# may-/joeys2t

Measured on AMD Instinct MI355X. Metric: audio frames/sec (train step, 80-mel, 15 s utt, bs32 per GPU), higher is better.
Workload: dtype bf16; 1 GPU; configs/librispeech_100h.yaml ASR train step on synthetic 16 kHz waveforms; global_batch=32, frames_per_utt=1498, encoder_len=375, lengths=fixed 15 s, vocab=5000, batch_multiplier=1, parallelism=dp1, launch=hipGraph replay

## Files before the change

include/joeys2t_hip.h:

```cpp
#ifndef JOEYS2T_HIP_H
#define JOEYS2T_HIP_H

#include <stdint.h>

#ifdef __cplusplus
extern "C" {
#endif

typedef void* js2t_stream;

enum { JS2T_F32 = 0, JS2T_BF16 = 1, JS2T_FP8_E4M3 = 2  };
enum { JS2T_ACT_NONE = 0, JS2T_ACT_RELU = 1, JS2T_ACT_GELU = 2, JS2T_ACT_SWISH = 3, JS2T_ACT_TANH = 4, JS2T_ACT_HARDSWISH = 5 };
enum { JS2T_OK = 0, JS2T_ERR_INVALID = -1, JS2T_ERR_LAUNCH = -2, JS2T_ERR_UNSUPPORTED = -3 };

int js2t_abi_version(void);
const char* js2t_last_error(void);

typedef struct js2t_gemm_desc {
  int32_t M, N, K;
  int32_t batch, batch_inner;
  int32_t dtype_ab, dtype_c;
  int32_t trans_a, trans_b;
  const void* A; int64_t lda, a_stride_o, a_stride_i;
  const void* B; int64_t ldb, b_stride_o, b_stride_i;
// ... 43 lines not shown
void js2t_gemm_p192_mode(int mode);
void js2t_gemm_wg256_mode(int mode);
void js2t_gemm_p192_ring(int nst);
void js2t_gemm_panel_mode(int mode);


int js2t_axpby(const void* x, float a, const void* y, float b, void* out, int64_t n, int dt, js2t_stream stream);

int js2t_cast(const void* src, int src_dt, void* dst, int dst_dt, int64_t n, js2t_stream stream);

int js2t_fold_ln_weights(const int64_t* table, int32_t n_entries, int32_t max_rows, js2t_stream stream);

int js2t_absmax(const void* x, int dt, int64_t n, float* out, js2t_stream stream);
int js2t_quantize_fp8(const void* x, int dt, void* y, int64_t n, const float* amax, const float* mul, float* scale_out,
                      js2t_stream stream);
int js2t_quantize_fp8_delayed(const void* x, int dt, void* y, int64_t n, float* state, const float* mul, float* scale_out,
                              js2t_stream stream);

int js2t_glu_fwd(const void* x, void* y, int64_t rows, int64_t C, int dt, js2t_stream stream);
int js2t_glu_bwd(const void* x, const void* dy, void* dx, int64_t rows, int64_t C, int dt, js2t_stream stream);
int js2t_glu_fwd_crop(const void* x, void* y, int64_t rows, int64_t C, int64_t T, const int64_t* valid_t, int dt, js2t_stream stream);
int js2t_glu_bwd_crop(const void* x, const void* dy, void* dx, int64_t rows, int64_t C, int64_t T, const int64_t* valid_t, int dt,
                      js2t_stream stream);

int js2t_transpose_groups(const void* src, void* dst, const int64_t* table, int32_t n_groups, int64_t total_tiles, js2t_stream stream);

int js2t_add_pe_dropout(const void* x, const float* pe, const void* extra, void* y, int64_t B, int64_t T,
                        int64_t D, int dt, float p, const uint64_t* rng_state, uint32_t rng_stream,
                        js2t_stream stream);

int js2t_dropout_bwd(const void* dy, void* dx, int64_t rows, int64_t cols, int dt, float p,
                     const uint64_t* rng_state, uint32_t rng_stream, js2t_stream stream);

int js2t_act_bwd(const void* dh, const void* z, void* dz, int64_t n, int act, int dt, float scale,
                 js2t_stream stream);

int js2t_embed_fwd(const int64_t* ids, const void* table, int table_dt, void* out, int out_dt,
                   int64_t n_ids, int64_t D, int64_t vocab, float scale, js2t_stream stream);
int js2t_embed_bwd(const int64_t* ids, const void* dout, int dout_dt, float* dtable, int64_t n_ids,
                   int64_t D, int64_t vocab, float scale, int64_t pad_idx, js2t_stream stream);

int64_t js2t_colsum_partial_rows(int64_t rows);
int js2t_colsum(const void* x, int dt, float* out, float* partial, int64_t rows, int64_t cols, int accumulate,
                js2t_stream stream);

int js2t_pack_rows(const void* src, void* dst, const int32_t* seg, int32_t B, int32_t T, int64_t rows_out, int64_t row_bytes,
// ... 212 lines not shown
```

joeys2t_amd/builders.py:

```python
from typing import Callable

from torch import nn


class ConfigurationError(Exception):
    """Custom exception for misspecifications of configuration (reference config.py:22)."""


class _Tanh(nn.Module):
    def forward(self, x):
        raise RuntimeError("placeholder activation module: the HIP GEMM epilogue applies tanh")


_ACTIVATIONS = {"relu": nn.ReLU, "gelu": nn.GELU, "tanh": _Tanh, "swish": nn.SiLU}


def build_activation(activation: str = "relu") -> Callable:
    try:
        return _ACTIVATIONS[activation]
    except KeyError:
        raise ConfigurationError("Invalid activation function. Valid options: " + ", ".join(repr(k) for k in _ACTIVATIONS) + ".") from None


import ctypes as _C
# ... 129 lines not shown
                    _C.c_float(g["weight_decay"]), _C.c_int64(self.t), ops._p(coef), _C.c_float(grad_scale), int(zero_grad),
                    ops._p(lr_dev), ops._p(step_dev), ops._stream())
            for table, n_items, n_units in plan["launches"]:
                check(lib().js2t_adamw_items(ops._p(st.flat), ops._p(st.flat_grad), ops._p(self.exp_avg), ops._p(self.exp_avg_sq),
                                             ops._p(lp), ops._p(st.flat_lp_t if lp is not None else None), ops._p(table),
                                             _C.c_int32(n_items), _C.c_int64(n_units), ops._p(plan["folds"]), *args), "js2t_adamw_items")
            ops.WEIGHT_VERSION += 1
            st.dirty = lp is None and st.dirty
            if plan["left_folds"] is not None:
                ops.fold_ln_weights(plan["left_folds"], plan["left_folds"].shape[0], plan["left_max_rows"])
            return
        for lo, hi in self.update_ranges:
            check(lib().js2t_adamw(_off(st.flat, lo), _off(st.flat_grad, lo), _off(self.exp_avg, lo), _off(self.exp_avg_sq, lo),
                                   _off(lp, lo), _C.c_int64(hi - lo), _C.c_float(g["lr"]), _C.c_float(g["betas"][0]),
                                   _C.c_float(g["betas"][1]), _C.c_float(g["eps"]), _C.c_float(g["weight_decay"]), _C.c_int64(self.t),
                                   ops._p(coef), _C.c_float(grad_scale), int(zero_grad), ops._p(lr_dev), ops._p(step_dev),
                                   ops._stream()), "js2t_adamw")
        ops.WEIGHT_VERSION += 1
        st.dirty = lp is None and st.dirty
        if lp is not None and st.flat_lp_t is not None:
            st.refresh_t()
        if lp is not None:
            st.refresh_folds()

    def _fused_plan(self):
        st = self.store
        if not FUSED_UPDATE or self.update_ranges != [(0, st.total)]:
            return None
        key = (len(st._fold_rows), st.flat_lp is not None, st.flat_lp_t is not None, None if self.keep is None else self.keep.version)
        if self._plan_key == key:
            return self._plan
        if torch.cuda.is_current_stream_capturing():
            raise RuntimeError("FlatAdamW: the store changed (new LayerNorm folds / shadows) after the last eager update: "
                               "run one eager step before capturing")
        if self._plan is not None:
            self._retired_plans.append(self._plan)
            self.plan_generation += 1
        self._plan_key, self._plan = key, None
        from joeys2t_amd._lib import lib
        geo = [_C.c_int32() for _ in range(3)]
        lib().js2t_adamw_items_geometry(*[_C.byref(v) for v in geo])
        flat_unit, unit_rows, unit_cols = (int(v.value) for v in geo)
        mats = sorted((off, R, Cc) for off, R, Cc, _ in st._tgroups)
        if any(Cc % 4 or off % 4 for off, R, Cc in mats):
            return None
        base = st.flat.data_ptr()
        fold_of, left = {}, []
        for i, row in enumerate(st._fold_rows):
            hit = [(off, R, Cc) for off, R, Cc in mats if base + 4 * off == row[0] and R == row[6] and Cc == row[7]]
            if hit and row[7] <= unit_cols and hit[0][0] not in fold_of:
                fold_of[hit[0][0]] = i
            else:
                left.append(row)
        small, big, pos = [], [], 0
        for off, R, Cc in mats:
            if off > pos:
                small.append([0, pos, off - pos, 1, 0, -1, 0, 0])
            kept = int(self.keep is not None and self.keep.contains(off, off + R * Cc))
            big.append([1, off, R, Cc, 0, fold_of.get(off, -1), kept, 0])
            pos = off + R * Cc
        if st.total > pos:
            small.append([0, pos, st.total - pos, 1, 0, -1, 0, 0])
        launches = []
        for items in (small, big):
            if not items:
                continue
            units = 0
            for it in items:
                it[4] = units
                units += -(-it[2] // flat_unit) if it[0] == 0 else -(-it[2] // unit_rows) * -(-it[3] // unit_cols)
            launches.append((torch.tensor(items, dtype=torch.int64, device=st.device), len(items), units))
        folds = torch.tensor(st._fold_rows, dtype=torch.int64, device=st.device) if st._fold_rows else None
        self._plan = {"launches": launches, "folds": folds,
                      "left_folds": torch.tensor(left, dtype=torch.int64, device=st.device) if left else None,
                      "left_max_rows": max((r[6] for r in left), default=0)}
        return self._plan

    def state_dict(self) -> Dict:
        return {"t": self.t, "exp_avg": self.exp_avg, "exp_avg_sq": self.exp_avg_sq, "param_groups": self.param_groups}

    def load_state_dict(self, sd: Dict):
        self.t = sd["t"]
        self.exp_avg.copy_(sd["exp_avg"])
        self.exp_avg_sq.copy_(sd["exp_avg_sq"])
        self.param_groups = sd["param_groups"]
        self.step_dev.fill_(self.t)
        self.lr_dev.fill_(self.param_groups[0]["lr"])

    def torch_state_dict(self, params) -> Dict:
        st = self.store
        state = {}
        if self.t > 0:
            for i, p in enumerate(params):
# ... 59 lines not shown
```

joeys2t_amd/csrc/elementwise.hip:

```cpp
#include "common.hpp"

namespace {

constexpr int EW_THREADS = 256;
inline int ew_grid(int64_t work_items) {
  int64_t g = (work_items + EW_THREADS - 1) / EW_THREADS;
  if (g < 1) g = 1;
  if (g > 4096) g = 4096;
  return (int)g;
}

template <typename T> struct vec4;
template <> struct vec4<float> {
  static __device__ __forceinline__ void ld(const float* p, float (&v)[4]) {
    const float4 x = *(const float4*)p; v[0] = x.x; v[1] = x.y; v[2] = x.z; v[3] = x.w;
  }
  static __device__ __forceinline__ void st(float* p, const float (&v)[4]) {
    *(float4*)p = make_float4(v[0], v[1], v[2], v[3]);
  }
};
template <> struct vec4<uint16_t> {
  static __device__ __forceinline__ void ld(const uint16_t* p, float (&v)[4]) {
    const uint2 x = *(const uint2*)p;
    v[0] = __uint_as_float(x.x << 16); v[1] = __uint_as_float(x.x & 0xffff0000u);
    v[2] = __uint_as_float(x.y << 16); v[3] = __uint_as_float(x.y & 0xffff0000u);
  }
  static __device__ __forceinline__ void st(uint16_t* p, const float (&v)[4]) {
    uint2 x;
    x.x = pack_bf16x2(v[0], v[1]);
    x.y = pack_bf16x2(v[2], v[3]);
    *(uint2*)p = x;
  }
};

template <typename S, typename D>
__global__ void cast_kernel(const S* __restrict__ src, D* __restrict__ dst, int64_t n) {
  const int64_t n4 = n >> 2;
  for (int64_t i = blockIdx.x * (int64_t)blockDim.x + threadIdx.x; i < n4; i += (int64_t)gridDim.x * blockDim.x) {
    float v[4];
    vec4<S>::ld(src + 4 * i, v);
    vec4<D>::st(dst + 4 * i, v);
  }
  for (int64_t i = (n4 << 2) + blockIdx.x * (int64_t)blockDim.x + threadIdx.x; i < n; i += (int64_t)gridDim.x * blockDim.x)
    io<D>::st(dst + i, io<S>::ld(src + i));
}

template <typename T>
__global__ void axpby_kernel(const T* __restrict__ x, float a, const T* __restrict__ y, float b, T* __restrict__ out,
                             int64_t n) {
  for (int64_t i = blockIdx.x * (int64_t)blockDim.x + threadIdx.x; i < n; i += (int64_t)gridDim.x * blockDim.x) {
    float v = a * io<T>::ld(x + i);
    if (y) v += b * io<T>::ld(y + i);
    io<T>::st(out + i, v);
  }
}

// ... 142 lines not shown
  const int cl = threadIdx.x & 63, sub = threadIdx.x >> 6;
  const int64_t c = ((int64_t)blockIdx.x * 64 + cl) * 8;
  const int64_t r0 = (int64_t)blockIdx.y * CS_ROWS_PER_BLOCK, r1 = min(rows, r0 + CS_ROWS_PER_BLOCK);
  float s[8] = {0.f, 0.f, 0.f, 0.f, 0.f, 0.f, 0.f, 0.f};
  if (c < cols)
    for (int64_t r = r0 + sub; r < r1; r += 4) {
      const uint4 v = *(const uint4*)(x + r * cols + c);
      const uint32_t vv[4] = {v.x, v.y, v.z, v.w};
#pragma unroll
      for (int i = 0; i < 4; ++i) {
        s[2 * i] += __uint_as_float(vv[i] << 16);
        s[2 * i + 1] += __uint_as_float(vv[i] & 0xffff0000u);
      }
    }
#pragma unroll
  for (int i = 0; i < 8; ++i) sh[sub][cl][i] = s[i];
  __syncthreads();
  if (sub == 0 && c < cols) {
#pragma unroll
    for (int i = 0; i < 8; ++i)
      partial[(int64_t)blockIdx.y * cols + c + i] = (sh[0][cl][i] + sh[1][cl][i]) + (sh[2][cl][i] + sh[3][cl][i]);
  }
}
__global__ __launch_bounds__(256) void colsum_final_kernel(const float* __restrict__ partial, float* __restrict__ out, int64_t nparts,
                                                           int64_t cols, int accumulate) {
  __shared__ float sh[4][64];
  const int cl = threadIdx.x & 63, sub = threadIdx.x >> 6;
  const int64_t c = (int64_t)blockIdx.x * 64 + cl;
  float s0 = 0.f, s1 = 0.f;
  if (c < cols) {
    int64_t p = sub;
    for (; p + 4 < nparts; p += 8) {
      s0 += partial[p * cols + c];
      s1 += partial[(p + 4) * cols + c];
    }
    for (; p < nparts; p += 4) s0 += partial[p * cols + c];
  }
  sh[sub][cl] = s0 + s1;
  __syncthreads();
  if (sub == 0 && c < cols) {
    const float tot = (sh[0][cl] + sh[1][cl]) + (sh[2][cl] + sh[3][cl]);
    out[c] = accumulate ? out[c] + tot : tot;
  }
}

template <typename D>
// ... 259 lines not shown
                           js2t_stream stream) {
  if (cols == 0) return JS2T_OK;
  if (rows == 0) {
    JS2T_CHECK(out, "colsum: bad arguments");
    if (!accumulate) {
      hipError_t e = hipMemsetAsync(out, 0, sizeof(float) * cols, (hipStream_t)stream);
      JS2T_CHECK(e == hipSuccess, "colsum: memset failed: %s", hipGetErrorString(e));
    }
    return JS2T_OK;
  }
  JS2T_CHECK(x && out && partial && rows > 0, "colsum: bad arguments");
  const int64_t nparts = js2t_colsum_partial_rows(rows);
  JS2T_CHECK(nparts <= 65535, "colsum: too many rows");
  hipStream_t s = (hipStream_t)stream;
  if (dt == JS2T_BF16 && cols % 8 == 0 && (((uintptr_t)x) & 15) == 0) {
    hipLaunchKernelGGL(colsum_partial_vec_kernel, dim3(cdiv(cols, 512), (unsigned)nparts), dim3(256), 0, s, (const uint16_t*)x,
                       partial, rows, cols);
  } else {
    const dim3 g1(cdiv(cols, 64), (unsigned)nparts);
    DISPATCH_DT(dt, T, hipLaunchKernelGGL((colsum_partial_kernel<T>), g1, dim3(256), 0, s, (const T*)x, partial, rows, cols));
  }
  JS2T_LAUNCH_CHECK();
  hipLaunchKernelGGL(colsum_final_kernel, dim3(cdiv(cols, 64)), dim3(256), 0, s, partial, out, nparts, cols, accumulate);
  JS2T_LAUNCH_CHECK();
  return JS2T_OK;
}

extern "C" int js2t_conv_weight_pack(const float* w, void* wp, int wp_dt, int64_t cout, int64_t cin, int64_t k,
                                     js2t_stream stream) {
  JS2T_CHECK(w && wp && cout > 0 && cin > 0 && k > 0, "conv_weight_pack: bad arguments");
  DISPATCH_DT(wp_dt, D, hipLaunchKernelGGL((conv_pack_kernel<D>), dim3(ew_grid(cout * cin * k)), dim3(EW_THREADS), 0,
                                           (hipStream_t)stream, w, (D*)wp, cout, cin, k));
  JS2T_LAUNCH_CHECK();
  return JS2T_OK;
}
extern "C" int js2t_conv_weight_unpack_grad(const float* dwp_t, float* dw, int64_t cout, int64_t cin, int64_t k,
                                            int accumulate, js2t_stream stream) {
  JS2T_CHECK(dwp_t && dw && cout > 0 && cin > 0 && k > 0, "conv_weight_unpack_grad: bad arguments");
  hipLaunchKernelGGL(conv_unpack_grad_kernel, dim3(ew_grid(cout * cin * k)), dim3(EW_THREADS), 0, (hipStream_t)stream, dwp_t,
                     dw, cout, cin, k, accumulate);
  JS2T_LAUNCH_CHECK();
  return JS2T_OK;
}
extern "C" int js2t_col2im(const void* dcol, void* dx, int64_t B, int64_t tin, int64_t tout, int64_t C, int64_t K,
                           int64_t stride, int64_t pad, int dt, js2t_stream stream) {
  if (B * tin * C == 0) return JS2T_OK;
// ... 271 lines not shown
```

joeys2t_amd/csrc/optim.hip:

```cpp
#include "common.hpp"

namespace {

constexpr int SQ_BLOCK = 256;
constexpr int SQ_PER_BLOCK = 256 * 16 * 4;

__global__ __launch_bounds__(SQ_BLOCK) void sumsq_partial_kernel(const float* __restrict__ x, int64_t n, float* __restrict__ partial) {
  __shared__ float red[SQ_BLOCK / 64];
  const int64_t base = (int64_t)blockIdx.x * SQ_PER_BLOCK;
  const int64_t end = min(n, base + SQ_PER_BLOCK);
  float s = 0.f;
  for (int64_t i = base + threadIdx.x * 4; i < end; i += SQ_BLOCK * 4) {
    if (i + 4 <= end) {
      const float4 v = *(const float4*)(x + i);
      s += v.x * v.x + v.y * v.y + v.z * v.z + v.w * v.w;
    } else {
      for (int64_t j = i; j < end; ++j) s += x[j] * x[j];
    }
  }
  s = block_sum(s, red);
  if (threadIdx.x == 0) partial[blockIdx.x] = s;
}


// ... 93 lines not shown
                                                          float wd, float bc1, float bc2_sqrt, const float* __restrict__ gscale_dev,
                                                          float gscale, int zero_grad, const float* __restrict__ lr_dev,
                                                          const int64_t* __restrict__ step_dev) {
  extern __shared__ __attribute__((aligned(16))) uint16_t tile[];
  AdamConsts k;
  k.gs = gscale * (gscale_dev ? *gscale_dev : 1.f);
  if (lr_dev) lr = *lr_dev;
  if (step_dev) {
    const double t = (double)(*step_dev);
    bc1 = (float)(1.0 - pow((double)b1, t));
    bc2_sqrt = (float)sqrt(1.0 - pow((double)b2, t));
  }
  k.lr = lr, k.b1 = b1, k.b2 = b2, k.eps = eps, k.wd = wd, k.bc2_sqrt = bc2_sqrt, k.step_size = lr / bc1;
  const int64_t bid = blockIdx.x;
  int lo = 0, hi = n_items - 1;
  while (lo < hi) {
    const int mid = (lo + hi + 1) >> 1;
    if (items[mid * 8 + 4] <= bid) lo = mid; else hi = mid - 1;
  }
  const int64_t* it = items + 8 * lo;
  const int64_t kind = it[0], off = it[1], R = it[2], Cc = it[3], u = bid - it[4], fold = it[5];
  if (it[6]) zero_grad = 0;
  const float4 zero4 = make_float4(0.f, 0.f, 0.f, 0.f);
  if (kind == 0) {
    const int64_t base = off + u * ADAM_FLAT, end = min(off + R, base + (int64_t)ADAM_FLAT);
    for (int64_t i = base + threadIdx.x * 4; i < end; i += 1024) {
      const float4 pv = *(float4*)(p + i), gv = *(float4*)(g + i), mv = *(float4*)(m + i), vv = *(float4*)(v + i);
      float pa[4] = {pv.x, pv.y, pv.z, pv.w}, ma[4] = {mv.x, mv.y, mv.z, mv.w}, va[4] = {vv.x, vv.y, vv.z, vv.w};
      adam4(pa, gv, ma, va, k);
      *(float4*)(p + i) = make_float4(pa[0], pa[1], pa[2], pa[3]);
      *(float4*)(m + i) = make_float4(ma[0], ma[1], ma[2], ma[3]);
      *(float4*)(v + i) = make_float4(va[0], va[1], va[2], va[3]);
      if (zero_grad) *(float4*)(g + i) = zero4;
      if (lp) *(uint2*)(lp + i) = make_uint2(pack_bf16x2(pa[0], pa[1]), pack_bf16x2(pa[2], pa[3]));
    }
    return;
  }
  const int64_t chunks = (Cc + ADAM_COLS - 1) / ADAM_COLS;
  const int64_t strip = u / chunks, r0 = strip * ADAM_ROWS, c0 = (u - strip * chunks) * ADAM_COLS;
  const int wave = threadIdx.x >> 6, lane = threadIdx.x & 63;
  const int64_t* fe = (fold >= 0 && chunks == 1) ? folds + 8 * fold : nullptr;
  float4 gam[2] = {zero4, zero4}, bet[2] = {zero4, zero4};
  if (fe) {
#pragma unroll
    for (int j = 0; j < 2; ++j) {
      const int64_t c = 4 * lane + 256 * j;
      if (c < Cc) gam[j] = *(const float4*)((const float*)fe[1] + c), bet[j] = *(const float4*)((const float*)fe[2] + c);
    }
  }
#pragma unroll 2
  for (int rr = 0; rr < ADAM_ROWS / 4; ++rr) {
    const int lr_ = wave * (ADAM_ROWS / 4) + rr;
    const int64_t r = r0 + lr_;
    if (r >= R) break;
    float pn[2][4];
    float cs = 0.f, bs = 0.f;
#pragma unroll
// ... 137 lines not shown
```

joeys2t_amd/encoders.py:

```python
import os
from typing import List, Tuple

import torch
from torch import Tensor, nn

from joeys2t_amd import functional as Fn
from joeys2t_amd import ops
from joeys2t_amd.helpers import freeze_params, lengths_to_padding_mask, pad
from joeys2t_amd.runtime import runtime_of
from joeys2t_amd.transformer_layers import ConformerEncoderLayer, PositionalEncoding, TransformerEncoderLayer


PACK_RAGGED = os.environ.get("JS2T_PACKED_ENCODER", "1") != "0"
PACK_MIN_SAVING = 0.04
PACK_ROUND = 64
_PACK_CACHE: dict = {}


class Encoder(nn.Module):

    @property
    def output_size(self):
        return self._output_size

# ... 12 lines not shown
    def get_out_seq_lens_tensor(self, in_seq_lens_tensor: Tensor) -> Tensor:
        out = in_seq_lens_tensor.long()
        for k in self.kernel_sizes:
            out = torch.div(out + 2 * (k // 2) - k, 2, rounding_mode="floor") + 1
        return out

    def out_len(self, t_in: int) -> int:
        for k in self.kernel_sizes:
            t_in = Fn.conv_out_len(t_in, k)
        return t_in

    def forward(self, src_tokens: Tensor, src_lengths: Tensor, crop: Tensor = None) -> Tuple[Tensor, Tensor, Tensor]:
        rt = runtime_of(self)
        if not src_lengths.is_cuda:
            max_len = int(src_lengths.max())
            assert max_len > 0, "empty batch!"
            if src_tokens.size(1) != max_len:
                src_tokens = src_tokens[:, :max_len, :]
            src_lengths = src_lengths.to(src_tokens.device)
        x = rt.act_in(src_tokens.contiguous())
        for i, conv in enumerate(self.conv_layers):
            valid = crop[i:i + 1] if (crop is not None and i + 1 < self.n_layers) else None
            x = Fn.Conv1dGluFn.apply(x, conv.weight, conv.bias, rt.compute_dtype,
                                     rt.sinks({"w": [conv.weight], "b": [conv.bias]}), rt.grads_ready, valid)
        out_lens, mask = ops.subsample_lengths_mask(src_lengths, x.size(1), self.kernel_sizes)
        mask.js2t_row_sums = out_lens
        return x, out_lens, mask


class TransformerEncoder(Encoder):

    def __init__(self, hidden_size: int = 512, ff_size: int = 2048, num_layers: int = 8, num_heads: int = 4,
                 dropout: float = 0.1, emb_dropout: float = 0.1, freeze: bool = False, **kwargs):
        super().__init__()
        self._output_size = hidden_size
        self.layers = nn.ModuleList([
            TransformerEncoderLayer(size=hidden_size, ff_size=ff_size, num_heads=num_heads, dropout=dropout,
                                    alpha=kwargs.get("alpha", 1.0), layer_norm=kwargs.get("layer_norm", "pre"),
                                    activation=kwargs.get("activation", "relu")) for _ in range(num_layers)
        ])
        self.pe = PositionalEncoding(hidden_size)
        self.emb_dropout = nn.Dropout(p=emb_dropout)
        self.layer_norm = nn.LayerNorm(hidden_size, eps=1e-6) if kwargs.get("layer_norm", "post") == "pre" else None
        if freeze:
            freeze_params(self)
        self.subsample = kwargs.get("subsample", False)
        if self.subsample:
# ... 110 lines not shown
```

joeys2t_amd/functional.py:

```python
import math
from typing import List, Optional

import os

import torch

from joeys2t_amd import ops
from joeys2t_amd.ops import DropoutRng

LN_EPS = 1e-6


def _row_major_2d(t: torch.Tensor) -> torch.Tensor:
    if t.dim() != 2 or t.stride(1) != 1:
        raise ops.Js2tError(f"expected a row-major 2-D tensor, got shape {tuple(t.shape)} strides {t.stride()}")
    return t


FP8_FORWARD = os.environ.get("JS2T_FP8_FORWARD", "0") == "1"
FP8_SEPARATE_PASS = os.environ.get("JS2T_FP8_SEPARATE_PASS", "0") == "1"
_FP8_WEIGHTS = {}
_FP8_STATES = {}
FP8_DELAYED = os.environ.get("JS2T_FP8_DELAYED", "1") != "0"

# ... 840 lines not shown

        dz, dw2, db2 = linear_bwd(dy2, z, w2c, dw_out=sv("w2", w2c), db_out=sink.get("b2"), queue=sink.get("_wq"))
        dv, dgamma, dbeta = ops.bn_act_bwd(dz, v2, gamma, beta, mean, invstd, training, "hardswish")
        du, dwd = ops.dwconv_outer_bwd(dv.view(B, T, -1), u.view(B, T, -1), wd2)
        dbd = ops.colsum(dv)
        dh = ops.glu_bwd(h, du.view(B * T, -1))
        dx, dw1, db1 = linear_bwd(dh, x2, w1c, dw_out=sv("w1", w1c), db_out=sink.get("b1"), queue=sink.get("_wq"))
        if sink and ctx.notify is not None:
            ctx.notify(ctx.leaves)
        dx = dx.view(B, T, Cc)
        if dx.dtype != in_dtype:
            dx = dx.to(in_dtype)
        return (dx, None if dw1 is None else dw1.view(dw1.shape[0], Cc, 1), db1, dwd.view(dwd.shape[0], 1, -1), dbd, dgamma, dbeta, None, None,
                None if dw2 is None else dw2.view(dw2.shape[0], -1, 1), db2, None, None, None, None, None, None, None, None)


def conv_out_len(t_in: int, k: int, stride: int = 2) -> int:
    return (t_in + 2 * (k // 2) - (k - 1) - 1) // stride + 1


class Conv1dGluFn(torch.autograd.Function):

    @staticmethod
    def forward(ctx, x, weight, bias, compute_dtype, sink=None, notify=None, valid_t=None):
        ctx.sink, ctx.notify, ctx.leaves = sink, notify, (weight, bias)
        ctx.valid_t = valid_t
        B, T, Cin = x.shape
        Cout, _, K = weight.shape
        stride, pad = 2, K // 2
        Tout = conv_out_len(T, K, stride)
        x = x.contiguous()
        wp = ops.conv_weight_pack(weight, compute_dtype)
        M = B * Tout
        pre = torch.empty((M, Cout), dtype=compute_dtype, device=x.device)
        conv = (T, Tout, Cin, stride, pad)
        vec = 8 if x.dtype == torch.bfloat16 else 4
        if Cin % vec == 0:
            col = ops.im2col(x, K, stride, pad, Tout)
            ops.gemm(col, wp, pre, M=M, N=Cout, K=K * Cin, lda=K * Cin, ldb=K * Cin, ldc=Cout, bias=bias)
        else:
            col = None
            ops.gemm(x, wp, pre, M=M, N=Cout, K=K * Cin, lda=stride * Cin, ldb=K * Cin, ldc=Cout, bias=bias, conv=conv)
        y = ops.glu_fwd(pre, Tout, valid_t)
        ctx.x, ctx.wp, ctx.pre, ctx.conv, ctx.col = (x if col is None else None), wp, pre, conv, col
        ctx.dims = (B, T, Cin, Cout, K, Tout)
        return y.view(B, Tout, Cout // 2)

    @staticmethod
    def backward(ctx, dy):
        B, T, Cin, Cout, K, Tout = ctx.dims
        M = B * Tout
        x, wp, pre, conv = ctx.x, ctx.wp, ctx.pre, ctx.conv
        dy2 = dy.reshape(M, Cout // 2)
        if not dy2.is_contiguous():
            dy2 = dy2.contiguous()
        dpre = ops.glu_bwd(pre, dy2, Tout, ctx.valid_t)
        sink = ctx.sink or {}
        db = ops.colsum(dpre, out=sink.get("b"), accumulate=True) if sink else ops.colsum(dpre)
        sk = wgrad_split(K * Cin, Cout, M)
        dwp_t = (torch.zeros if sk > 1 else torch.empty)((K * Cin, Cout), dtype=torch.float32, device=dpre.device)
        if ctx.col is not None:
            ops.gemm(ctx.col, dpre, dwp_t, M=K * Cin, N=Cout, K=M, lda=K * Cin, ldb=Cout, ldc=Cout, trans_a=True, trans_b=True, split_k=sk)
        else:
            ops.gemm(x, dpre, dwp_t, M=K * Cin, N=Cout, K=M, lda=conv[3] * Cin, ldb=Cout, ldc=Cout, trans_a=True, trans_b=True,
                     conv=conv, split_k=sk)
        dw = ops.conv_weight_unpack_grad(dwp_t, Cout, Cin, K, out=sink.get("w"))
        if sink:
            if ctx.notify is not None:
                ctx.notify(ctx.leaves)
            dw = db = None
        dx = None
        if ctx.needs_input_grad[0]:
            dcol = torch.empty((M, K * Cin), dtype=pre.dtype, device=pre.device)
            ops.gemm(dpre, wp, dcol, M=M, N=K * Cin, K=Cout, lda=Cout, ldb=K * Cin, ldc=K * Cin, trans_b=True)
            dx = ops.col2im(dcol, B, T, Tout, Cin, K, conv[3], conv[4])
        return dx, dw, db, None, None, None, None
```

joeys2t_amd/ops.py:

```python
import ctypes as C
import math
from typing import Optional, Sequence

import torch

from joeys2t_amd._lib import ACT_CODES, BF16, F32, AttnDesc, GemmDesc, Js2tError, check, lib

FP8 = 2
_DT = {torch.float32: F32, torch.bfloat16: BF16, torch.float8_e4m3fn: FP8}


def dt_code(t_or_dtype) -> int:
    dtype = t_or_dtype.dtype if torch.is_tensor(t_or_dtype) else t_or_dtype
    try:
        return _DT[dtype]
    except KeyError:
        raise Js2tError(f"unsupported dtype {dtype}: the HIP path computes in float32 or bfloat16") from None


def _dev(*tensors):
    for t in tensors:
        if t is not None and not t.is_cuda:
            raise Js2tError(
                "joeys2t_amd ops run on the GPU through libjoeys2t_hip.so only; got a CPU tensor "
# ... 221 lines not shown

def transpose_groups(src, dst, table, n_groups: int, total_tiles: int):
    _dev(src, dst, table)
    check(lib().js2t_transpose_groups(_p(src), _p(dst), _p(table), int(n_groups), C.c_int64(total_tiles), _stream()), "js2t_transpose_groups")


def glu_fwd(x: torch.Tensor, T: Optional[int] = None, valid_t: Optional[torch.Tensor] = None) -> torch.Tensor:
    _dev(x, valid_t)
    rows, c2 = x.shape[0], x.shape[1]
    y = torch.empty((rows, c2 // 2), dtype=x.dtype, device=x.device)
    check(lib().js2t_glu_fwd_crop(_p(x), _p(y), C.c_int64(rows), C.c_int64(c2 // 2), C.c_int64(T if valid_t is not None else max(rows, 1)),
                                  _p(valid_t), dt_code(x), _stream()), "js2t_glu_fwd")
    return y


def glu_bwd(x: torch.Tensor, dy: torch.Tensor, T: Optional[int] = None, valid_t: Optional[torch.Tensor] = None) -> torch.Tensor:
    _dev(x, dy, valid_t)
    dx = torch.empty_like(x)
    check(lib().js2t_glu_bwd_crop(_p(x), _p(dy), _p(dx), C.c_int64(x.shape[0]), C.c_int64(x.shape[1] // 2),
                                  C.c_int64(T if valid_t is not None else max(x.shape[0], 1)), _p(valid_t), dt_code(x), _stream()), "js2t_glu_bwd")
    return dx


def add_pe_dropout(x, pe, extra, p, rng: Optional[DropoutRng], site: int):
    _dev(x, pe, extra)
    B, T, D = x.shape
    y = torch.empty_like(x)
    check(lib().js2t_add_pe_dropout(_p(x), _p(pe), _p(extra), _p(y), C.c_int64(B), C.c_int64(T), C.c_int64(D), dt_code(x),
                                    C.c_float(p), _p(rng.state) if p > 0 else None, C.c_uint32(site), _stream()),
          "js2t_add_pe_dropout")
    return y


def dropout_bwd(dy, p, rng: DropoutRng, site: int):
    _dev(dy)
    dy = dy.contiguous()
    cols = dy.shape[-1]
    rows = dy.numel() // cols
    dx = torch.empty_like(dy)
    check(lib().js2t_dropout_bwd(_p(dy), _p(dx), C.c_int64(rows), C.c_int64(cols), dt_code(dy), C.c_float(p),
                                 _p(rng.state), C.c_uint32(site), _stream()), "js2t_dropout_bwd")
    return dx


def act_bwd(dh, z, act: str, scale: float = 1.0):
    _dev(dh, z)
# ... 17 lines not shown
    _dev(ids, dout, out)
    ids, dout = ids.contiguous(), dout.contiguous()
    D = dout.shape[-1]
    dtable = out if out is not None else torch.zeros((vocab, D), dtype=torch.float32, device=dout.device)
    check(lib().js2t_embed_bwd(_p(ids), _p(dout), dt_code(dout), _p(dtable), C.c_int64(ids.numel()), C.c_int64(D),
                               C.c_int64(vocab), C.c_float(scale), C.c_int64(-1 if pad_idx is None else pad_idx), _stream()),
          "js2t_embed_bwd")
    return dtable


def colsum(x2d: torch.Tensor, out: Optional[torch.Tensor] = None, accumulate: bool = False) -> torch.Tensor:
    _dev(x2d, out)
    rows, cols = x2d.shape
    if out is None:
        out = torch.empty((cols,), dtype=torch.float32, device=x2d.device)
        accumulate = False
    nparts = lib().js2t_colsum_partial_rows(rows)
    partial = torch.empty((max(nparts, 1) * cols,), dtype=torch.float32, device=x2d.device)
    check(lib().js2t_colsum(_p(x2d), dt_code(x2d), _p(out), _p(partial), C.c_int64(rows), C.c_int64(cols), int(accumulate),
                            _stream()), "js2t_colsum")
    return out


def conv_weight_pack(w: torch.Tensor, dtype) -> torch.Tensor:
    _dev(w)
    cout, cin, k = w.shape
    wp = torch.empty((cout, k * cin), dtype=dtype, device=w.device)
    check(lib().js2t_conv_weight_pack(_p(w.contiguous()), _p(wp), dt_code(wp), C.c_int64(cout), C.c_int64(cin), C.c_int64(k),
                                      _stream()), "js2t_conv_weight_pack")
    return wp


def conv_weight_unpack_grad(dwp_t: torch.Tensor, cout: int, cin: int, k: int, out: Optional[torch.Tensor] = None) -> torch.Tensor:
    _dev(dwp_t, out)
    acc = out is not None
    dw = out if acc else torch.empty((cout, cin, k), dtype=torch.float32, device=dwp_t.device)
    check(lib().js2t_conv_weight_unpack_grad(_p(dwp_t), _p(dw), C.c_int64(cout), C.c_int64(cin), C.c_int64(k), int(acc),
                                             _stream()), "js2t_conv_weight_unpack_grad")
    return dw


def im2col(x3d, K, stride, pad, tout):
    _dev(x3d)
    B, tin, Cc = x3d.shape
    x3d = x3d.contiguous()
    col = torch.empty((B * tout, K * Cc), dtype=x3d.dtype, device=x3d.device)
    check(lib().js2t_im2col(_p(x3d), _p(col), C.c_int64(B), C.c_int64(tin), C.c_int64(tout), C.c_int64(Cc), C.c_int64(K),
                            C.c_int64(stride), C.c_int64(pad), dt_code(x3d), _stream()), "js2t_im2col")
    return col

# ... 663 lines not shown
```

joeys2t_amd/runtime.py:

```python
from typing import Dict, List, Optional, Sequence, Tuple

import torch
from torch import nn

from joeys2t_amd import ops

_ALIGN = 64


class ParamStore:

    def __init__(self, module: nn.Module, device: torch.device):
        self.device = torch.device(device)
        group_of: Dict[int, List[nn.Parameter]] = {}
        for m in module.modules():
            fg = getattr(m, "fuse_groups", None)
            if fg is None:
                continue
            for grp in fg():
                grp = [p for p in grp if p is not None]
                if any(id(p) in group_of for p in grp):
                    continue
                for p in grp:
                    group_of[id(p)] = grp
# ... 40 lines not shown
                cur_key, cur_lo = k, boundary
            total = (total + _ALIGN - 1) // _ALIGN * _ALIGN
            for p in grp:
                offsets[id(p)] = total
                total += p.numel()
        total = (total + _ALIGN - 1) // _ALIGN * _ALIGN
        if total > cur_lo:
            self.type_ranges.append((cur_lo, total))
            if cur_key != "prefix" and cur_key[0] == 1:
                self.late_ranges.append((cur_lo, total))
        self.total = total
        self.offsets = offsets
        self.params: List[nn.Parameter] = [p for grp in groups for p in grp]
        self._tgroups: List[Tuple[int, int, int, List[nn.Parameter]]] = []
        self._tgroup_of: Dict[int, int] = {}
        for grp in groups:
            if all(p.dim() == 2 for p in grp) and len({p.shape[1] for p in grp}) == 1 and grp[0].shape[1] % 4 == 0:
                rows = sum(p.shape[0] for p in grp)
                for p in grp:
                    self._tgroup_of[id(p)] = len(self._tgroups)
                self._tgroups.append((offsets[id(grp[0])], rows, grp[0].shape[1], list(grp)))
        self.flat_lp_t: Optional[torch.Tensor] = None
        self._ttable = None
        self.flat = torch.zeros(total, dtype=torch.float32, device=self.device)
        self.flat_grad = torch.zeros(total, dtype=torch.float32, device=self.device)
        self.flat_lp: Optional[torch.Tensor] = None
        self.dirty = True
        self.auto_refresh = True
        with torch.no_grad():
            for p in self.params:
                off, n = offsets[id(p)], p.numel()
                view = self.flat[off:off + n].view(p.shape)
                view.copy_(p.data.to(device=self.device, dtype=torch.float32))
                p.data = view
                p.grad = None
        self._cache: Dict[Tuple, torch.Tensor] = {}
        self._folds: Dict[Tuple, LnFold] = {}
        self._fold_rows: List[List[int]] = []
        self._retired_fold_tables: List[torch.Tensor] = []
        self._fold_table: Optional[torch.Tensor] = None
        self._fold_max_rows = 0

    def fold(self, weights: Sequence[nn.Parameter], biases: Sequence[nn.Parameter], gamma: nn.Parameter, beta: nn.Parameter):
        key = tuple(id(p) for p in (*weights, *biases, gamma, beta))
        hit = self._folds.get(key)
        if hit is not None:
# ... 43 lines not shown
        except KeyError:
            return None
        base_ptr = self.flat_grad.data_ptr()
        for i, p in enumerate(params):
            if not p.requires_grad or p.grad is None or p.grad.data_ptr() != base_ptr + 4 * offs[i]:
                return None
            if i and (offs[i] != offs[i - 1] + params[i - 1].numel() or p.shape[1:] != params[0].shape[1:]):
                return None
        rows = sum(p.shape[0] for p in params)
        n = sum(p.numel() for p in params)
        return self.flat_grad[offs[0]:offs[0] + n].view(rows, *params[0].shape[1:])

    def refresh(self, force: bool = False):
        if self.flat_lp is None:
            self.flat_lp = torch.empty(self.total, dtype=torch.bfloat16, device=self.device)
            self._cache.clear()
            force = True
        if force or self.dirty:
            ops.cast(self.flat, torch.bfloat16, out=self.flat_lp)
            self.dirty = False
            if self.flat_lp_t is not None:
                self.refresh_t()
            self.refresh_folds()

    def refresh_t(self):
        if self.flat_lp is None:
            self.refresh()
        if self.flat_lp_t is None:
            self.flat_lp_t = torch.zeros(self.total, dtype=torch.bfloat16, device=self.device)
            rows, t0 = [], 0
            for off, R, Cc, _ in self._tgroups:
                rows.append([off, R, Cc, t0])
                t0 += ((R + 63) // 64) * ((Cc + 63) // 64)
            self._ttable = (torch.tensor(rows, dtype=torch.int64, device=self.device), len(rows), t0)
            self._cache_t: Dict[Tuple, torch.Tensor] = {}
        table, n, tiles = self._ttable
        ops.transpose_groups(self.flat_lp, self.flat_lp_t, table, n, tiles)

    def view_t(self, params: Sequence[nn.Parameter]) -> Optional[torch.Tensor]:
        gi = self._tgroup_of.get(id(params[0]))
        if gi is None or any(self._tgroup_of.get(id(p)) != gi for p in params):
            return None
        if self.flat_lp_t is None:
            self.refresh_t()
        key = tuple(id(p) for p in params)
        hit = self._cache_t.get(key)
        if hit is not None:
            return hit
        off, R, Cc, members = self._tgroups[gi]
        r0 = (self.offsets[id(params[0])] - off) // Cc
        rows = sum(p.shape[0] for p in params)
        for a, b in zip(params[:-1], params[1:]):
            if self.offsets[id(b)] != self.offsets[id(a)] + a.numel():
                return None
        out = self.flat_lp_t[off:off + R * Cc].view(Cc, R)[:, r0:r0 + rows]
        self._cache_t[key] = out
        return out

    def mark_dirty(self):
        self.dirty = True

    def view(self, params: Sequence[nn.Parameter], dtype: torch.dtype) -> Optional[torch.Tensor]:
        key = (tuple(id(p) for p in params), dtype)
        hit = self._cache.get(key)
        if hit is not None:
            return hit
        try:
            offs = [self.offsets[id(p)] for p in params]
        except KeyError:
            return None
        for i in range(1, len(params)):
            if offs[i] != offs[i - 1] + params[i - 1].numel() or params[i].shape[1:] != params[0].shape[1:]:
                return None
        rows = sum(p.shape[0] for p in params)
        n = sum(p.numel() for p in params)
        if dtype == torch.float32:
            base = self.flat
        else:
            if self.flat_lp is None:
                self.refresh()
# ... 171 lines not shown
        return self._side_stream

    def weight(self, params: Sequence[nn.Parameter]) -> torch.Tensor:
        dt = self.compute_dtype
        if self.store is not None:
            v = self.store.view(params, dt)
            if v is not None:
                return v
        ws = []
        for p in params:
            ws.append(p.data if p.dtype == dt else ops.cast(p.data, dt))
        return ws[0] if len(ws) == 1 else torch.cat(ws, dim=0)

    def ln_fold(self, weights, biases, ln: Optional[nn.LayerNorm]) -> Optional[LnFold]:
        if ln is None or self.store is None or self.compute_dtype != torch.bfloat16 or any(b is None for b in biases):
            return None
        return self.store.fold(weights, biases, ln.weight, ln.bias)

    def weight_t(self, params: Sequence[nn.Parameter]) -> Optional[torch.Tensor]:
        if self.store is None or self.compute_dtype != torch.bfloat16 or not torch.is_grad_enabled():
            return None
        return self.store.view_t(params)

    def bias(self, params: Sequence[Optional[nn.Parameter]]) -> Optional[torch.Tensor]:
        if any(p is None for p in params):
            return None
        if self.store is not None:
            v = self.store.view(params, torch.float32)
            if v is not None:
                return v
        bs = [p.data for p in params]
        return bs[0] if len(bs) == 1 else torch.cat(bs, dim=0)

    def grad_sink(self, params: Sequence[Optional[nn.Parameter]]) -> Optional[torch.Tensor]:
        if self.store is None or not self.direct_grads or any(p is None for p in params):
            return None
        return self.store.grad_view(params)

    def sinks(self, mapping) -> Optional[dict]:
        if not torch.is_grad_enabled():
            return None
        out = {}
        for name, ps in mapping.items():
            v = self.grad_sink(ps)
            if v is None:
                return None
# ... 37 lines not shown
```

Measured before the change: 4.385 million frames/s.

## Fuse GLU backward with bias colsum and persist packed conv weights via optimizer

Adds a fused GLU-backward kernel that writes dx and accumulates per-block column partial sums for the conv bias gradient in one pass. This removes the separate colsum read of dpre. It also keeps a persistent bf16 packed copy of each conv weight, which the fused AdamW kernel writes directly (new item kind 2). That removes the per-step conv_weight_pack launch in forward. In exchange the optimizer does scattered 2-byte stores for the conv items, and the pack only exists once an eager (non-captured) step has built it.

```diff
diff --git a/include/joeys2t_hip.h b/include/joeys2t_hip.h
--- a/include/joeys2t_hip.h
+++ b/include/joeys2t_hip.h
@@ -89,6 +89,8 @@
 int js2t_glu_fwd_crop(const void* x, void* y, int64_t rows, int64_t C, int64_t T, const int64_t* valid_t, int dt, js2t_stream stream);
 int js2t_glu_bwd_crop(const void* x, const void* dy, void* dx, int64_t rows, int64_t C, int64_t T, const int64_t* valid_t, int dt,
                       js2t_stream stream);
+int js2t_glu_bwd_colsum(const void* x, const void* dy, void* dx, float* db, float* partial, int64_t rows, int64_t C, int64_t T,
+                        const int64_t* valid_t, int dt, int accumulate, js2t_stream stream);
 
 int js2t_transpose_groups(const void* src, void* dst, const int64_t* table, int32_t n_groups, int64_t total_tiles, js2t_stream stream);
 
diff --git a/joeys2t_amd/builders.py b/joeys2t_amd/builders.py
--- a/joeys2t_amd/builders.py
+++ b/joeys2t_amd/builders.py
@@ -175,12 +175,14 @@
             st.refresh_t()
         if lp is not None:
             st.refresh_folds()
+            st.refresh_conv_packs()
 
     def _fused_plan(self):
         st = self.store
         if not FUSED_UPDATE or self.update_ranges != [(0, st.total)]:
             return None
-        key = (len(st._fold_rows), st.flat_lp is not None, st.flat_lp_t is not None, None if self.keep is None else self.keep.version)
+        key = (len(st._fold_rows), st.flat_lp is not None, st.flat_lp_t is not None, None if self.keep is None else self.keep.version,
+               len(st._conv_packs))
         if self._plan_key == key:
             return self._plan
         if torch.cuda.is_current_stream_capturing():
@@ -205,15 +207,27 @@
                 fold_of[hit[0][0]] = i
             else:
                 left.append(row)
+        convs = sorted((st.offsets[id(w)], w.numel(), w.shape[1], w.shape[2], wp.data_ptr()) for w, wp in st._conv_packs.values())
         small, big, pos = [], [], 0
+
+        def flat_items(lo, hi):
+            for off, n, cin, k, ptr in convs:
+                if lo <= off and off + n <= hi:
+                    if off > lo:
+                        small.append([0, lo, off - lo, 1, 0, -1, 0, 0])
+                    small.append([2, off, n, cin, 0, k, 0, ptr])
+                    lo = off + n
+            if hi > lo:
+                small.append([0, lo, hi - lo, 1, 0, -1, 0, 0])
+
         for off, R, Cc in mats:
             if off > pos:
-                small.append([0, pos, off - pos, 1, 0, -1, 0, 0])
+                flat_items(pos, off)
             kept = int(self.keep is not None and self.keep.contains(off, off + R * Cc))
             big.append([1, off, R, Cc, 0, fold_of.get(off, -1), kept, 0])
             pos = off + R * Cc
         if st.total > pos:
-            small.append([0, pos, st.total - pos, 1, 0, -1, 0, 0])
+            flat_items(pos, st.total)
         launches = []
         for items in (small, big):
             if not items:
@@ -221,7 +235,7 @@
             units = 0
             for it in items:
                 it[4] = units
-                units += -(-it[2] // flat_unit) if it[0] == 0 else -(-it[2] // unit_rows) * -(-it[3] // unit_cols)
+                units += -(-it[2] // flat_unit) if it[0] != 1 else -(-it[2] // unit_rows) * -(-it[3] // unit_cols)
             launches.append((torch.tensor(items, dtype=torch.int64, device=st.device), len(items), units))
         folds = torch.tensor(st._fold_rows, dtype=torch.int64, device=st.device) if st._fold_rows else None
         self._plan = {"launches": launches, "folds": folds,
diff --git a/joeys2t_amd/csrc/elementwise.hip b/joeys2t_amd/csrc/elementwise.hip
--- a/joeys2t_amd/csrc/elementwise.hip
+++ b/joeys2t_amd/csrc/elementwise.hip
@@ -32,6 +32,10 @@
     *(uint2*)p = x;
   }
 };
+
+template <typename T> __device__ __forceinline__ float rounded(float v);
+template <> __device__ __forceinline__ float rounded<float>(float v) { return v; }
+template <> __device__ __forceinline__ float rounded<uint16_t>(float v) { return bf16_bits_to_f32(f32_to_bf16_bits(v)); }
 
 template <typename S, typename D>
 __global__ void cast_kernel(const S* __restrict__ src, D* __restrict__ dst, int64_t n) {
@@ -220,6 +224,49 @@
       partial[(int64_t)blockIdx.y * cols + c + i] = (sh[0][cl][i] + sh[1][cl][i]) + (sh[2][cl][i] + sh[3][cl][i]);
   }
 }
+template <typename T>
+__global__ __launch_bounds__(256) void glu_bwd_colsum_kernel(const T* __restrict__ x, const T* __restrict__ dy, T* __restrict__ dx,
+                                                             float* __restrict__ partial, int64_t rows, int64_t C, int64_t T_,
+                                                             const int64_t* __restrict__ valid_t) {
+  __shared__ float sh[4][64][9];
+  const int cl = threadIdx.x & 63, sub = threadIdx.x >> 6;
+  const int64_t c = ((int64_t)blockIdx.x * 64 + cl) * 4, vt = valid_t ? *valid_t : T_;
+  const int64_t r0 = (int64_t)blockIdx.y * CS_ROWS_PER_BLOCK, r1 = min(rows, r0 + CS_ROWS_PER_BLOCK);
+  float s[8] = {0.f, 0.f, 0.f, 0.f, 0.f, 0.f, 0.f, 0.f};
+  if (c < C) {
+#pragma unroll 4
+    for (int64_t r = r0 + sub; r < r1; r += 4) {
+      float a[4], b[4], g[4], da[4], db[4];
+      vec4<T>::ld(x + r * 2 * C + c, a);
+      vec4<T>::ld(x + r * 2 * C + C + c, b);
+      vec4<T>::ld(dy + r * C + c, g);
+      const bool live = (r % T_) < vt;
+#pragma unroll
+      for (int i = 0; i < 4; ++i) {
+        const float gi = live ? g[i] : 0.f;
+        const float sg = 1.f / (1.f + __expf(-b[i]));
+        da[i] = rounded<T>(gi * sg);
+        db[i] = rounded<T>(gi * a[i] * sg * (1.f - sg));
+        s[i] += da[i];
+        s[4 + i] += db[i];
+      }
+      vec4<T>::st(dx + r * 2 * C + c, da);
+      vec4<T>::st(dx + r * 2 * C + C + c, db);
+    }
+  }
+#pragma unroll
+  for (int i = 0; i < 8; ++i) sh[sub][cl][i] = s[i];
+  __syncthreads();
+  if (sub == 0 && c < C) {
+    float* out = partial + (int64_t)blockIdx.y * 2 * C + c;
+#pragma unroll
+    for (int i = 0; i < 4; ++i) {
+      out[i] = (sh[0][cl][i] + sh[1][cl][i]) + (sh[2][cl][i] + sh[3][cl][i]);
+      out[C + i] = (sh[0][cl][4 + i] + sh[1][cl][4 + i]) + (sh[2][cl][4 + i] + sh[3][cl][4 + i]);
+    }
+  }
+}
+
 __global__ __launch_bounds__(256) void colsum_final_kernel(const float* __restrict__ partial, float* __restrict__ out, int64_t nparts,
                                                            int64_t cols, int accumulate) {
   __shared__ float sh[4][64];
@@ -525,6 +572,26 @@
   }
   JS2T_LAUNCH_CHECK();
   hipLaunchKernelGGL(colsum_final_kernel, dim3(cdiv(cols, 64)), dim3(256), 0, s, partial, out, nparts, cols, accumulate);
+  JS2T_LAUNCH_CHECK();
+  return JS2T_OK;
+}
+
+extern "C" int js2t_glu_bwd_colsum(const void* x, const void* dy, void* dx, float* db, float* partial, int64_t rows, int64_t C, int64_t T_,
+                                   const int64_t* valid_t, int dt, int accumulate, js2t_stream stream) {
+  if (rows * C == 0) return JS2T_OK;
+  JS2T_CHECK(x && dy && dx && db && partial && rows > 0 && C > 0 && T_ > 0 && rows % T_ == 0, "glu_bwd_colsum: bad arguments");
+  const int64_t nparts = js2t_colsum_partial_rows(rows);
+  JS2T_CHECK(nparts <= 65535, "glu_bwd_colsum: too many rows");
+  const int esz = dt == JS2T_F32 ? 4 : 2;
+  if ((C & 3) || ((((uintptr_t)x) | ((uintptr_t)dy) | ((uintptr_t)dx)) & (uintptr_t)(4 * esz - 1))) {
+    const int rc = js2t_glu_bwd_crop(x, dy, dx, rows, C, T_, valid_t, dt, stream);
+    return rc != JS2T_OK ? rc : js2t_colsum(dx, dt, db, partial, rows, 2 * C, accumulate, stream);
+  }
+  hipStream_t s = (hipStream_t)stream;
+  DISPATCH_DT(dt, T, hipLaunchKernelGGL((glu_bwd_colsum_kernel<T>), dim3(cdiv(C, 256), (unsigned)nparts), dim3(256), 0, s, (const T*)x,
+                                        (const T*)dy, (T*)dx, partial, rows, C, T_, valid_t));
+  JS2T_LAUNCH_CHECK();
+  hipLaunchKernelGGL(colsum_final_kernel, dim3(cdiv(2 * C, 64)), dim3(256), 0, s, partial, db, nparts, 2 * C, accumulate);
   JS2T_LAUNCH_CHECK();
   return JS2T_OK;
 }
diff --git a/joeys2t_amd/csrc/optim.hip b/joeys2t_amd/csrc/optim.hip
--- a/joeys2t_amd/csrc/optim.hip
+++ b/joeys2t_amd/csrc/optim.hip
@@ -139,7 +139,9 @@
   const int64_t kind = it[0], off = it[1], R = it[2], Cc = it[3], u = bid - it[4], fold = it[5];
   if (it[6]) zero_grad = 0;
   const float4 zero4 = make_float4(0.f, 0.f, 0.f, 0.f);
-  if (kind == 0) {
+  if (kind == 0 || kind == 2) {
+    uint16_t* pack = kind == 2 ? (uint16_t*)it[7] : nullptr;
+    const int64_t cin = Cc, kw_n = fold, ck = cin * kw_n;
     const int64_t base = off + u * ADAM_FLAT, end = min(off + R, base + (int64_t)ADAM_FLAT);
     for (int64_t i = base + threadIdx.x * 4; i < end; i += 1024) {
       const float4 pv = *(float4*)(p + i), gv = *(float4*)(g + i), mv = *(float4*)(m + i), vv = *(float4*)(v + i);
@@ -150,6 +152,13 @@
       *(float4*)(v + i) = make_float4(va[0], va[1], va[2], va[3]);
       if (zero_grad) *(float4*)(g + i) = zero4;
       if (lp) *(uint2*)(lp + i) = make_uint2(pack_bf16x2(pa[0], pa[1]), pack_bf16x2(pa[2], pa[3]));
+      if (pack) {
+#pragma unroll
+        for (int e = 0; e < 4; ++e) {
+          const int64_t j = i - off + e, o = j / ck, rem = j - o * ck, c = rem / kw_n, kw = rem - c * kw_n;
+          pack[o * ck + kw * cin + c] = f32_to_bf16_bits(pa[e]);
+        }
+      }
     }
     return;
   }
diff --git a/joeys2t_amd/encoders.py b/joeys2t_amd/encoders.py
--- a/joeys2t_amd/encoders.py
+++ b/joeys2t_amd/encoders.py
@@ -58,7 +58,7 @@
         for i, conv in enumerate(self.conv_layers):
             valid = crop[i:i + 1] if (crop is not None and i + 1 < self.n_layers) else None
             x = Fn.Conv1dGluFn.apply(x, conv.weight, conv.bias, rt.compute_dtype,
-                                     rt.sinks({"w": [conv.weight], "b": [conv.bias]}), rt.grads_ready, valid)
+                                     rt.sinks({"w": [conv.weight], "b": [conv.bias]}), rt.grads_ready, valid, rt.conv_weight(conv.weight))
         out_lens, mask = ops.subsample_lengths_mask(src_lengths, x.size(1), self.kernel_sizes)
         mask.js2t_row_sums = out_lens
         return x, out_lens, mask
diff --git a/joeys2t_amd/functional.py b/joeys2t_amd/functional.py
--- a/joeys2t_amd/functional.py
+++ b/joeys2t_amd/functional.py
@@ -886,7 +886,7 @@
 class Conv1dGluFn(torch.autograd.Function):
 
     @staticmethod
-    def forward(ctx, x, weight, bias, compute_dtype, sink=None, notify=None, valid_t=None):
+    def forward(ctx, x, weight, bias, compute_dtype, sink=None, notify=None, valid_t=None, wp=None):
         ctx.sink, ctx.notify, ctx.leaves = sink, notify, (weight, bias)
         ctx.valid_t = valid_t
         B, T, Cin = x.shape
@@ -894,7 +894,8 @@
         stride, pad = 2, K // 2
         Tout = conv_out_len(T, K, stride)
         x = x.contiguous()
-        wp = ops.conv_weight_pack(weight, compute_dtype)
+        if wp is None:
+            wp = ops.conv_weight_pack(weight, compute_dtype)
         M = B * Tout
         pre = torch.empty((M, Cout), dtype=compute_dtype, device=x.device)
         conv = (T, Tout, Cin, stride, pad)
@@ -918,9 +919,8 @@
         dy2 = dy.reshape(M, Cout // 2)
         if not dy2.is_contiguous():
             dy2 = dy2.contiguous()
-        dpre = ops.glu_bwd(pre, dy2, Tout, ctx.valid_t)
         sink = ctx.sink or {}
-        db = ops.colsum(dpre, out=sink.get("b"), accumulate=True) if sink else ops.colsum(dpre)
+        dpre, db = ops.glu_bwd_colsum(pre, dy2, Tout, ctx.valid_t, db_out=sink.get("b"))
         sk = wgrad_split(K * Cin, Cout, M)
         dwp_t = (torch.zeros if sk > 1 else torch.empty)((K * Cin, Cout), dtype=torch.float32, device=dpre.device)
         if ctx.col is not None:
@@ -938,4 +938,4 @@
             dcol = torch.empty((M, K * Cin), dtype=pre.dtype, device=pre.device)
             ops.gemm(dpre, wp, dcol, M=M, N=K * Cin, K=Cout, lda=Cout, ldb=K * Cin, ldc=K * Cin, trans_b=True)
             dx = ops.col2im(dcol, B, T, Tout, Cin, K, conv[3], conv[4])
-        return dx, dw, db, None, None, None, None
+        return dx, dw, db, None, None, None, None, None
diff --git a/joeys2t_amd/ops.py b/joeys2t_amd/ops.py
--- a/joeys2t_amd/ops.py
+++ b/joeys2t_amd/ops.py
@@ -267,6 +267,21 @@
     return dx
 
 
+def glu_bwd_colsum(x, dy, T: Optional[int] = None, valid_t: Optional[torch.Tensor] = None, db_out: Optional[torch.Tensor] = None):
+    _dev(x, dy, valid_t, db_out)
+    rows, c2 = x.shape
+    if rows == 0:
+        dx = torch.empty_like(x)
+        return dx, colsum(dx, out=db_out, accumulate=True)
+    dx = torch.empty_like(x)
+    db = db_out if db_out is not None else torch.empty((c2, ), dtype=torch.float32, device=x.device)
+    partial = torch.empty((max(lib().js2t_colsum_partial_rows(rows), 1) * c2, ), dtype=torch.float32, device=x.device)
+    check(lib().js2t_glu_bwd_colsum(_p(x), _p(dy), _p(dx), _p(db), _p(partial), C.c_int64(rows), C.c_int64(c2 // 2),
+                                    C.c_int64(T if valid_t is not None else max(rows, 1)), _p(valid_t), dt_code(x), int(db_out is not None),
+                                    _stream()), "js2t_glu_bwd_colsum")
+    return dx, db
+
+
 def add_pe_dropout(x, pe, extra, p, rng: Optional[DropoutRng], site: int):
     _dev(x, pe, extra)
     B, T, D = x.shape
@@ -330,10 +345,10 @@
     return out
 
 
-def conv_weight_pack(w: torch.Tensor, dtype) -> torch.Tensor:
-    _dev(w)
+def conv_weight_pack(w: torch.Tensor, dtype, out: Optional[torch.Tensor] = None) -> torch.Tensor:
+    _dev(w, out)
     cout, cin, k = w.shape
-    wp = torch.empty((cout, k * cin), dtype=dtype, device=w.device)
+    wp = out if out is not None else torch.empty((cout, k * cin), dtype=dtype, device=w.device)
     check(lib().js2t_conv_weight_pack(_p(w.contiguous()), _p(wp), dt_code(wp), C.c_int64(cout), C.c_int64(cin), C.c_int64(k),
                                       _stream()), "js2t_conv_weight_pack")
     return wp
diff --git a/joeys2t_amd/runtime.py b/joeys2t_amd/runtime.py
--- a/joeys2t_amd/runtime.py
+++ b/joeys2t_amd/runtime.py
@@ -86,6 +86,7 @@
                 self._tgroups.append((offsets[id(grp[0])], rows, grp[0].shape[1], list(grp)))
         self.flat_lp_t: Optional[torch.Tensor] = None
         self._ttable = None
+        self._conv_packs: Dict[int, Tuple[nn.Parameter, torch.Tensor]] = {}
         self.flat = torch.zeros(total, dtype=torch.float32, device=self.device)
         self.flat_grad = torch.zeros(total, dtype=torch.float32, device=self.device)
         self.flat_lp: Optional[torch.Tensor] = None
@@ -175,6 +176,7 @@
             if self.flat_lp_t is not None:
                 self.refresh_t()
             self.refresh_folds()
+            self.refresh_conv_packs()
 
     def refresh_t(self):
         if self.flat_lp is None:
@@ -209,6 +211,20 @@
         out = self.flat_lp_t[off:off + R * Cc].view(Cc, R)[:, r0:r0 + rows]
         self._cache_t[key] = out
         return out
+
+    def conv_packed(self, w: nn.Parameter) -> Optional[torch.Tensor]:
+        if self.flat_lp is None or w.dim() != 3 or w.numel() % 4 or id(w) not in self.offsets:
+            return None
+        hit = self._conv_packs.get(id(w))
+        if hit is None:
+            if torch.cuda.is_current_stream_capturing():
+                return None
+            hit = self._conv_packs[id(w)] = (w, ops.conv_weight_pack(w.data, torch.bfloat16))
+        return hit[1]
+
+    def refresh_conv_packs(self):
+        for w, wp in self._conv_packs.values():
+            ops.conv_weight_pack(w.data, torch.bfloat16, out=wp)
 
     def mark_dirty(self):
         self.dirty = True
@@ -426,6 +442,11 @@
             return None
         return self.store.view_t(params)
 
+    def conv_weight(self, w: nn.Parameter) -> Optional[torch.Tensor]:
+        if self.store is None or self.compute_dtype != torch.bfloat16 or not torch.is_grad_enabled():
+            return None
+        return self.store.conv_packed(w)
+
     def bias(self, params: Sequence[Optional[nn.Parameter]]) -> Optional[torch.Tensor]:
         if any(p is None for p in params):
             return None
```

Measured after the change: 4.391 million frames/s, median of 6. Within noise of the previous version (+0.1%).
